# postworthy/ghost

Measured on AMD Instinct MI355X. Metric: swapped frames/sec at 256×256 bf16, 1/2/4/8 MI355X; AAD decoder HBM GB/s, higher is better.
Workload: dtype bf16; 1 GPU; BASELINE config 2: batch=64 synthetic 256x256 aligned faces per GPU, AEI_Net unet num_blocks=2, faceshifter_batch (u8 in -> u8 out, device-resident; D2H in legs.d2h); global_batch=64, per_gpu_batch=64, backbone=unet, num_blocks=2, identities=1, parallelism=dp1, batches_in_flight=2

## Files before the change

ghost_amd/csrc/conv_halo.hip:

```cpp
#include <cstdio>
#include <cstdlib>
#include <type_traits>
#include <utility>

#include "conv_halo.h"
#include "ghost_common.h"
#include "plan_log.h"

namespace ghost {

template <int TH_, int TW_, int WM_, int WN_, int IMG_ = 1>
struct HaloCfg {
  static constexpr int TH = TH_, TW = TW_, WM = WM_, WN = WN_, IMG = IMG_;
  static constexpr int BN = 64 * WN, NW = WM * WN, WPI = WM / IMG;
  static constexpr int HWW = TW + 2, HHH = TH + 2;
  static constexpr int HIMG = HHH * HWW;
  static constexpr int HP = IMG * HIMG;
  static constexpr int HPIECES = (HP + 15) / 16;
  static constexpr int WPIECES = 9 * BN / 16;
  static constexpr int HALO_B = HPIECES * 1024;
  static constexpr int LDS_B = HALO_B + 9 * BN * 64;
  static constexpr int HPW = (HPIECES + NW - 1) / NW;
  static constexpr int WPW = (WPIECES + NW - 1) / NW;
  static_assert(IMG * TH * TW == 64 * WM, "each wave owns 64 output pixels");
// ... 408 lines not shown
    for (int i = 0; i < 4; ++i) acc[j][i] = f32x4{0.f, 0.f, 0.f, 0.f};

  constexpr bool W16 = !EPX && NCB == 2 && IMG == 1 && !(DBG & 16);
  constexpr int LPITCH = 136, LWAVE = 64 * LPITCH;
  constexpr bool LDSW = !EPX && !W16 && IMG == 1 && !RESW && !(DBG & 16) && STAGE_B >= NW * LWAVE;
  const bool plain = !a.scale && !a.shift && a.slope == 1.f && !a.tanh_out;
  constexpr int NST = ((DBG & 48) || EPX) ? 0 : ((W16 || LDSW) ? 8 : 16) + (STATS ? 1 : 0);
  if (nmine == 0) return;
  constexpr bool SPREAD = (DBG & 4096) == 0;
  constexpr int NPIECE = HPW + (RESW ? 0 : WPW);
  static_assert(NPIECE <= 16, "the spread-issue switch below has sixteen cases");
  constexpr int PPT = 2;
  Tile cur = tile_of(0);
  set_dma_tile(cur);
  issue(lds0, 0);
  __builtin_amdgcn_s_waitcnt(0x0F70);
  int k = 0;
  auto step = [&](const unsigned char* buf, unsigned char* nbuf, auto cbt) {
    constexpr int cb = decltype(cbt)::value;
    if constexpr (cb == 0)
      __builtin_amdgcn_s_waitcnt(((NST >> 4) << 14) | 0x0F70 | (NST & 15));
    else
      __builtin_amdgcn_s_waitcnt(0x0F70);
    __builtin_amdgcn_s_waitcnt(0xC07F);
    __builtin_amdgcn_s_barrier();
    const bool more = cb + 1 < NCB || k + 1 < nmine;
    if constexpr (cb + 1 < NCB) {
      if constexpr (!SPREAD) issue(nbuf, cb + 1);
    } else if (k + 1 < nmine) {
      set_dma_tile(tile_of(k + 1));
      if constexpr (!SPREAD) issue(nbuf, 0);
    }
    constexpr int ncb_next = cb + 1 < NCB ? cb + 1 : 0;
    const unsigned char* wb = RESW ? wres + cb * WBLK_B : buf + HALO_B;
    v8_t<T> wf[2][4], pf[2][4];
    auto load_frags = [&](int tap, v8_t<T> (&w)[4], v8_t<T> (&p)[4]) {
      const int dy = tap / 3, dx = tap - dy * 3;
#pragma unroll
      for (int j = 0; j < 4; ++j) {
        const int n = j * 16 + lr;
        w[j] = *reinterpret_cast<const v8_t<T>*>(wb + (tap * 64 + n) * 64 + ((lq ^ hswz(n)) * 16));
      }
#pragma unroll
      for (int i = 0; i < 4; ++i) {
        const int q = i * 16 + lr;
        const int P = G::himg(wid) + (G::hrow0(wid) + q / TW + dy) * HWW + q % TW + dx;
        p[i] = *reinterpret_cast<const v8_t<T>*>(buf + P * 64 + ((lq ^ hswz(P)) * 16));
      }
    };
    if constexpr ((DBG & 8) == 0) {
      load_frags(0, wf[0], pf[0]);
      if constexpr ((DBG & 64) != 0) load_frags(1, wf[1], pf[1]);
      asm volatile("" ::: "memory");
#pragma unroll
      for (int tap = 0; tap < 9; ++tap) {
        if constexpr ((DBG & 128) == 0) __builtin_amdgcn_s_waitcnt(0xC07F);
        if (tap + 1 < 9 && (DBG & 64) == 0) load_frags(tap + 1, wf[(tap + 1) & 1], pf[(tap + 1) & 1]);
#pragma unroll
        for (int j = 0; j < 4; ++j)
#pragma unroll
          for (int i = 0; i < 4; ++i)
            acc[j][i] = mfma16x16x32<T>(wf[tap & 1][j], pf[tap & 1][i], acc[j][i]);
        if constexpr (SPREAD) {
          if (more) {
            pp_unroll(std::make_integer_sequence<int, 16>{}, [&](auto qt) {
              constexpr int q = decltype(qt)::value;
              const int pc = tap * PPT + q;
              if ((q < PPT || (tap == 8 && pc < NPIECE)) && pc < NPIECE) {
                switch (pc) {
#define GHOST_SPREAD_CASE(N) case N: if constexpr (N < NPIECE) issue_piece(nbuf, ncb_next, std::integral_constant<int, N>{}); break;
                  GHOST_SPREAD_CASE(0) GHOST_SPREAD_CASE(1) GHOST_SPREAD_CASE(2) GHOST_SPREAD_CASE(3)
                  GHOST_SPREAD_CASE(4) GHOST_SPREAD_CASE(5) GHOST_SPREAD_CASE(6) GHOST_SPREAD_CASE(7)
                  GHOST_SPREAD_CASE(8) GHOST_SPREAD_CASE(9) GHOST_SPREAD_CASE(10) GHOST_SPREAD_CASE(11)
                  GHOST_SPREAD_CASE(12) GHOST_SPREAD_CASE(13) GHOST_SPREAD_CASE(14) GHOST_SPREAD_CASE(15)
#undef GHOST_SPREAD_CASE
                  default: break;
                }
              }
            });
          }
        }
        if constexpr ((DBG & 128) == 0) {
          if (tap + 1 < 9 && (DBG & 64) == 0) {
            __builtin_amdgcn_sched_group_barrier(0x100, 8, 0);
            __builtin_amdgcn_sched_group_barrier(0x008, 16, 0);
          } else {
            __builtin_amdgcn_sched_group_barrier(0x008, 16, 0);
          }
          __builtin_amdgcn_sched_barrier(0);
        } else {
          asm volatile("" ::: "memory");
        }
      }
    }
    if constexpr (cb + 1 < NCB) return;
    if constexpr ((DBG & 32) != 0) {
      float t = 0.f;
#pragma unroll
      for (int j = 0; j < 4; ++j)
#pragma unroll
        for (int i = 0; i < 4; ++i) {
          t += acc[j][i][0] + acc[j][i][1] + acc[j][i][2] + acc[j][i][3];
          acc[j][i] = f32x4{0.f, 0.f, 0.f, 0.f};
        }
      if (__float_as_uint(t) == 0x7fc00123u) ay_[lane] = (T)t;
      return;
    }
    unsigned char* stg = const_cast<unsigned char*>(buf) + wid * LWAVE;
    if constexpr (LDSW) {
      __builtin_amdgcn_s_waitcnt(0xC07F);
      __builtin_amdgcn_s_barrier();
    }
    auto epi_body = [&](auto mt) {
    constexpr int MODE = decltype(mt)::value;
    const bool has_res = MODE == 1 || (MODE == 0 && ares_ != nullptr);
    uint2 rraw[4][4];
    if (has_res) {
#pragma unroll
      for (int i = 0; i < 4; ++i) {
        const int q = i * 16 + lr;
        const int oy = cur.y0 + G::hrow0(wid) + q / TW, ox = cur.x0 + q % TW;
        const long pix = cur.base + (long)G::img(wid) * a.H * a.W + (long)oy * a.W + ox;
        const bool in = !EPX || (oy < a.H && ox < a.W);
#pragma unroll
        for (int j = 0; j < 4; ++j)
          rraw[i][j] = in ? *reinterpret_cast<const uint2*>(ares_ + pix * a.ldres + cur.n0 + j * 16 + lq * 4)
                          : make_uint2(0u, 0u);
      }
    }
#pragma unroll
    for (int i = 0; i < 4; ++i) {
      const int q = i * 16 + lr;
      const int oy = cur.y0 + G::hrow0(wid) + q / TW, ox = cur.x0 + q % TW;
      const long pix = cur.base + (long)G::img(wid) * a.H * a.W + (long)oy * a.W + ox;
      uint2 ov[4];
      if constexpr (EPX) {
        if (oy >= a.H || ox >= a.W) {
#pragma unroll
          for (int j = 0; j < 4; ++j) acc[j][i] = f32x4{0.f, 0.f, 0.f, 0.f};
          continue;
        }
      }
#pragma unroll
      for (int j = 0; j < 4; ++j) {
        const int n = cur.n0 + j * 16 + lq * 4;
        float rv[4] = {0.f, 0.f, 0.f, 0.f};
        if (has_res) {
          const T* e = reinterpret_cast<const T*>(&rraw[i][j]);
#pragma unroll
          for (int r = 0; r < 4; ++r) rv[r] = (float)e[r];
        }
        uint2 o;
        T* oe = reinterpret_cast<T*>(&o);
        if constexpr (EPX) {
          const f32x4 tsc = *reinterpret_cast<const f32x4*>(s_sc + n);
          const f32x4 tsh = *reinterpret_cast<const f32x4*>(s_sh + n);
          const f32x4 tpr = *reinterpret_cast<const f32x4*>(s_ex + n);
          float v[4];
#pragma unroll
          for (int r = 0; r < 4; ++r) {
            float t = fmaf(acc[j][i][r], tsc[r], tsh[r]);
            if (a.res_first) t += rv[r];
            t = t > 0.f ? t : t * tpr[r];
            if (!a.res_first) t += rv[r];
            if (a.tanh_out) t = tanhf(t);
            v[r] = t;
            oe[r] = (T)t;
            acc[j][i][r] = 0.f;
          }
          *reinterpret_cast<uint2*>(ay_ + pix * a.ldy + n) = o;
          if (ay2_) {
            const f32x4 tsc2 = *reinterpret_cast<const f32x4*>(s_ex + NMAX + n);
            const f32x4 tsh2 = *reinterpret_cast<const f32x4*>(s_ex + 2 * NMAX + n);
#pragma unroll
            for (int r = 0; r < 4; ++r) oe[r] = (T)(v[r] * tsc2[r] + tsh2[r]);
            *reinterpret_cast<uint2*>(ay2_ + pix * a.ldy2 + n) = o;
          }
        } else {
        float v[4];
        if constexpr (MODE != 0) {
#pragma unroll
          for (int r = 0; r < 4; ++r) v[r] = MODE == 1 ? acc[j][i][r] + rv[r] : acc[j][i][r];
        } else {
          const f32x4 tsc = *reinterpret_cast<const f32x4*>(s_sc + n);
          const f32x4 tsh = *reinterpret_cast<const f32x4*>(s_sh + n);
#pragma unroll
          for (int r = 0; r < 4; ++r) {
            float t = fmaf(acc[j][i][r], tsc[r], tsh[r]);
            t = t > 0.f ? t : t * a.slope;
            t += rv[r];
            if (a.tanh_out) t = tanhf(t);
            v[r] = t;
          }
        }
        o.x = pack2<T>(v[0], v[1]);
        o.y = pack2<T>(v[2], v[3]);
        if constexpr (STATS) {
          const f32x2 a01 = unpack2<T>(o.x), a23 = unpack2<T>(o.y);
          acc[j][i] = f32x4{a01.x, a01.y, a23.x, a23.y};
        } else {
          acc[j][i] = f32x4{0.f, 0.f, 0.f, 0.f};
        }
        if constexpr (W16) ov[j] = o;
        else if constexpr (LDSW) {
          *reinterpret_cast<uint2*>(stg + q * LPITCH + 32 * j + 8 * lq) = o;
        }
        else if constexpr (!(DBG & 16)) *reinterpret_cast<uint2*>(ay_ + pix * a.ldy + n) = o;
        else if ((o.x ^ o.y) == 0x7fc00001u) *reinterpret_cast<uint2*>(ay_ + pix * a.ldy + n) = o;
        }
      }
      if constexpr (W16) {
        uint2 a0, a1, b0, b1;
        {
          const auto x0 = __builtin_amdgcn_permlane16_swap(ov[0].x, ov[1].x, false, false);
          const auto y0 = __builtin_amdgcn_permlane16_swap(ov[0].y, ov[1].y, false, false);
          const auto x1 = __builtin_amdgcn_permlane16_swap(ov[2].x, ov[3].x, false, false);
          const auto y1 = __builtin_amdgcn_permlane16_swap(ov[2].y, ov[3].y, false, false);
          a0 = make_uint2(x0[0], y0[0]);
          a1 = make_uint2(x0[1], y0[1]);
          b0 = make_uint2(x1[0], y1[0]);
          b1 = make_uint2(x1[1], y1[1]);
        }
        static_assert(G::TW % 16 == 0, "a pixel fragment lies in one tile row");
        const long p0 = pix - lr + (lr & 7);
        store_rows16<T>(ay_ + cur.n0, p0 * a.ldy, (p0 + 8) * a.ldy, lr, (lq >> 1) + 2 * (lq & 1),
                        u32x4{a0.x, a0.y, a1.x, a1.y}, u32x4{b0.x, b0.y, b1.x, b1.y});
      }
    }
    };
    if constexpr (EPX) {
      epi_body(std::integral_constant<int, 0>{});
    } else {
      if (plain) {
        if (ares_) epi_body(std::integral_constant<int, 1>{});
        else epi_body(std::integral_constant<int, 2>{});
      } else {
        epi_body(std::integral_constant<int, 0>{});
      }
    }
    if constexpr (LDSW) {
      asm volatile("" ::: "memory");
      const int c = lane & 7, q0 = lane >> 3;
      T* __restrict__ yw = ay_ + (cur.base + (long)(cur.y0 + G::hrow0(wid)) * a.W + cur.x0) * a.ldy + cur.n0;
      const int lo = q0 * a.ldy + c * 8;
#pragma unroll
      for (int st = 0; st < 8; ++st) {
        const int q = 8 * st + q0;
        const u32x4 v = *reinterpret_cast<const u32x4*>(stg + q * LPITCH + c * 16);
        *reinterpret_cast<u32x4*>(yw + ((st >> 2) * a.W + 8 * (st & 3)) * a.ldy + lo) = v;
      }
    }
    if constexpr (STATS) {
      float S1, S2;
      tile_stats64_1p(acc, lr, S1, S2);
      const int c = cur.n0 + (lr >> 2) * 16 + lq * 4 + (lr & 3);
      float* dst;
      if constexpr (IMG > 1) {
        const long b = cur.base / ((long)a.H * a.W) + G::img(wid);
        dst = a.in_part + (b * (long)a.N + c) * 2;
      } else {
        const int tile = (cur.y0 / G::TH) * a.tiles_x + cur.x0 / TW;
        const long b = cur.base / ((long)a.H * a.W);
        dst = a.in_part + ((((b * a.tiles_x * a.tiles_y) + tile) * 8 + wid) * (long)a.N + c) * 2;
      }
      *reinterpret_cast<float2*>(dst) = make_float2(S1, S2);
    }
  };
  for (; k < nmine; ++k) {
    pp_unroll(std::make_integer_sequence<int, NCB / 2>{}, [&](auto pt) {
      constexpr int P = decltype(pt)::value;
      step(lds0, lds1, std::integral_constant<int, 2 * P>{});
      step(lds1, lds0, std::integral_constant<int, 2 * P + 1>{});
    });
    if (k + 1 < nmine) cur = tile_of(k + 1);
  }
  asm volatile("s_waitcnt vmcnt(0)" ::: "memory");
}

template <int BN>
struct HaloTCfg {
  static constexpr int TIH = 8, TIW = 16;
  static constexpr int HWW = TIW + 2, HP = (TIH + 2) * HWW;
  static constexpr int HPIECES = (HP + 15) / 16;
  static constexpr int WPIECES = 16 * BN / 16;
  static constexpr int HALO_B = HPIECES * 1024;
  static constexpr int LDS_B = HALO_B + 16 * BN * 64;
  static constexpr int NW = 8;
  static constexpr int HPW = (HPIECES + NW - 1) / NW;
  static constexpr int WPW = (WPIECES + NW - 1) / NW;
  static constexpr int TN = BN / 16;
};

struct HaloTArgs {
  const void* x;
  const void* w;
  void* y;
  const float* scale;
  const float* shift;
  const void* res;
  long wpar;
  int H, W, Cin, ldx, N, Kpad, ldy, ldres;
  float slope;
  int tiles_x, tiles_y, nNt;
};

template <typename T, int BN>
__global__ void __launch_bounds__(512) __attribute__((amdgpu_waves_per_eu(4, 8))) convT_halo_kernel(const HaloTArgs a) {
  const T* __restrict__ ax_ = reinterpret_cast<const T*>(a.x);
  const T* __restrict__ aw_ = reinterpret_cast<const T*>(a.w);
  T* __restrict__ ay_ = reinterpret_cast<T*>(a.y);
  const T* __restrict__ ares_ = reinterpret_cast<const T*>(a.res);
  using G = HaloTCfg<BN>;
  constexpr int HWW = G::HWW, HP = G::HP, HPIECES = G::HPIECES, WPIECES = G::WPIECES, HALO_B = G::HALO_B;
  constexpr int NWAVES = G::NW, HPW = G::HPW, WPW = G::WPW, TN = G::TN;
  __shared__ __attribute__((aligned(1024))) unsigned char lds[G::LDS_B];
  const int tid = threadIdx.x, lane = tid & 63, lr = lane & 15, lq = lane >> 4, wid = tid >> 6;
  const int ph = wid >> 1, py = ph >> 1, px = ph & 1, hf = wid & 1;
  int t = xcd_tile(blockIdx.x, gridDim.x);
  const int nt = t % a.nNt;
  t /= a.nNt;
  const int tx = t % a.tiles_x;
  t /= a.tiles_x;
  const int ty = t % a.tiles_y;
  const int b = t / a.tiles_y;
  const int y0 = ty * G::TIH, x0 = tx * G::TIW, n0 = nt * BN;
  const T* __restrict__ xs = ax_ + (long)b * a.H * a.W * a.ldx;

  const int prow = lane >> 2, slot = lane & 3;
  int h_off[HPW];
  unsigned h_ok = 0u;
#pragma unroll
  for (int j = 0; j < HPW; ++j) {
    const int piece = wid + j * NWAVES;
    const int P = piece * 16 + prow;
    const int hy = P / HWW, hx = P - hy * HWW;
    const int iy = y0 - 1 + hy, ix = x0 - 1 + hx;
    const bool ok = piece < HPIECES && P < HP && iy >= 0 && iy < a.H && ix >= 0 && ix < a.W;
    h_off[j] = ok ? (iy * a.W + ix) * a.ldx + ((slot ^ hswz(P)) * 8) : 0;
    h_ok |= (ok ? 1u : 0u) << j;
  }
  const T* wsrc[WPW];
#pragma unroll
  for (int j = 0; j < WPW; ++j) {
    const int piece = wid + j * NWAVES;
    const int pt = piece / (BN / 16), n = (piece % (BN / 16)) * 16 + prow;
    wsrc[j] = aw_ + (pt >> 2) * a.wpar + (long)(n0 + n) * a.Kpad + (pt & 3) * 32 + ((slot ^ hswz(n)) * 8);
  }

  f32x4 acc[TN][4];
#pragma unroll
  for (int j = 0; j < TN; ++j)
#pragma unroll
    for (int i = 0; i < 4; ++i) acc[j][i] = f32x4{0.f, 0.f, 0.f, 0.f};

  const int ncb = a.Cin / 32;
  for (int cb = 0; cb < ncb; ++cb) {
#if defined(__HIP_DEVICE_COMPILE__)
#pragma unroll
    for (int j = 0; j < HPW; ++j) {
      const int piece = wid + j * NWAVES;
      if (piece < HPIECES) {
        const void* src = ((h_ok >> j) & 1u) ? (const void*)(xs + h_off[j] + cb * 32) : (const void*)g_halo_zero;
        __builtin_amdgcn_global_load_lds(src, lds + piece * 1024, 16, 0, 0);
      }
    }
#pragma unroll
    for (int j = 0; j < WPW; ++j) {
      const int piece = wid + j * NWAVES;
      if (piece < WPIECES) __builtin_amdgcn_global_load_lds(wsrc[j] + cb * 128, lds + HALO_B + piece * 1024, 16, 0, 0);
    }
#endif
    asm volatile("s_waitcnt vmcnt(0)" ::: "memory");
    __syncthreads();
#pragma unroll
    for (int tp = 0; tp < 4; ++tp) {
      asm volatile("" ::: "memory");
      const int dy = py - (tp >> 1), dx = px - (tp & 1);
      v8_t<T> wf[TN], pf[4];
#pragma unroll
      for (int j = 0; j < TN; ++j) {
        const int n = j * 16 + lr;
        wf[j] = *reinterpret_cast<const v8_t<T>*>(lds + HALO_B + ((ph * 4 + tp) * BN + n) * 64 + ((lq ^ hswz(n)) * 16));
      }
#pragma unroll
      for (int i = 0; i < 4; ++i) {
        const int P = (hf * 4 + i + 1 + dy) * HWW + lr + 1 + dx;
        pf[i] = *reinterpret_cast<const v8_t<T>*>(lds + P * 64 + ((lq ^ hswz(P)) * 16));
      }
#pragma unroll
      for (int j = 0; j < TN; ++j)
#pragma unroll
        for (int i = 0; i < 4; ++i) acc[j][i] = mfma16x16x32<T>(wf[j], pf[i], acc[j][i]);
    }
    __syncthreads();
  }

  const int Wo = 2 * a.W, Ho = 2 * a.H;
#pragma unroll
  for (int i = 0; i < 4; ++i) {
    const int oy = 2 * (y0 + hf * 4 + i) + py, ox = 2 * (x0 + lr) + px;
    const long pix = ((long)b * Ho + oy) * Wo + ox;
#pragma unroll
    for (int j = 0; j < TN; ++j) {
      const int n = n0 + j * 16 + lq * 4;
      if (n >= a.N) continue;
      float rv[4] = {0.f, 0.f, 0.f, 0.f};
      if (ares_) {
        const uint2 raw = *reinterpret_cast<const uint2*>(ares_ + pix * a.ldres + n);
        const T* e = reinterpret_cast<const T*>(&raw);
#pragma unroll
        for (int r = 0; r < 4; ++r) rv[r] = (float)e[r];
      }
      uint2 o;
      T* oe = reinterpret_cast<T*>(&o);
#pragma unroll
      for (int r = 0; r < 4; ++r) {
        float v = acc[j][i][r];
        if (a.scale) v *= a.scale[n + r];
        if (a.shift) v += a.shift[n + r];
        v = v > 0.f ? v : v * a.slope;
        oe[r] = (T)(v + rv[r]);
      }
      *reinterpret_cast<uint2*>(ay_ + pix * a.ldy + n) = o;
    }
  }
}

bool convT_halo_supported(const ConvDesc& d) {
  static const int enabled = GHOST_KNOB("GHOST_CONVT_HALO", 1);
  if (!enabled || d.kind != CONV_T4S2 || !is16(d.ti) || d.to != d.ti || d.epi != EPI_STD) return false;
  if (d.u8 || d.tanh_out || d.force_split || d.Cin % 32 || d.ldx % 8 || d.ldy % 4 || (d.res && d.ldres % 4)) return false;
  if (d.res_first || d.prelu || d.y2) return false;
  if (d.Hi % HaloTCfg<64>::TIH || d.Wi % HaloTCfg<64>::TIW || d.Kpad < 4 * d.Cin) return false;
  if (!(d.N % 64 == 0 || d.N == 32) || d.Npad < d.N) return false;
  if ((uintptr_t)d.x % 16 || (uintptr_t)d.w % 16 || (uintptr_t)d.y % 8 || (d.res && (uintptr_t)d.res % 8)) return false;
  {
    const int bn = d.N == 32 ? 32 : 64;
    const long nt = (long)d.B * (d.Hi / HaloTCfg<64>::TIH) * (d.Wi / HaloTCfg<64>::TIW) * ((d.N + bn - 1) / bn);
    if (nt < 128) return false;
  }
  return (long)d.Hi * d.Wi * d.ldx < (1L << 31);
}

PlanSig convT_halo_signature(const ConvDesc& d) {
  PlanSig g;
  snprintf(g.s, sizeof(g.s), "convT_halo t=%s BN=%d Cin=%d N=%d res=%d", plan_dt(d.ti), d.N == 32 ? 32 : 64, d.Cin, d.N,
           d.res != nullptr);
  return g;
}

template <typename T, int BN>
static int haloT_launch(const ConvDesc& d, hipStream_t s) {
  HaloTArgs a{};
  a.x = d.x; a.w = d.w; a.y = d.y;
  a.scale = d.scale; a.shift = d.shift; a.res = d.res;
  a.wpar = (long)d.Npad * d.Kpad;
  a.H = d.Hi; a.W = d.Wi; a.Cin = d.Cin; a.ldx = d.ldx; a.N = d.N; a.Kpad = d.Kpad;
  a.ldy = d.ldy; a.ldres = d.ldres; a.slope = d.slope;
  a.tiles_x = d.Wi / HaloTCfg<BN>::TIW; a.tiles_y = d.Hi / HaloTCfg<BN>::TIH; a.nNt = (d.N + BN - 1) / BN;
  const long ntiles = (long)d.B * a.tiles_x * a.tiles_y * a.nNt;
  GHOST_PLAN_LOG("%s", convT_halo_signature(d).s);
  hipLaunchKernelGGL((convT_halo_kernel<T, BN>), dim3((unsigned)ntiles), dim3(512), 0, s, a);
  return (int)hipGetLastError();
}

int convT_halo(const ConvDesc& d, hipStream_t s) {
  if (!convT_halo_supported(d)) return -1;
  if (d.ti == GHOST_F16) return d.N == 32 ? haloT_launch<_Float16, 32>(d, s) : haloT_launch<_Float16, 64>(d, s);
  return d.N == 32 ? haloT_launch<bf16, 32>(d, s) : haloT_launch<bf16, 64>(d, s);
}

struct HaloGeom { int TH, TW, IMG, NW; const char* name; };
template <class G> static constexpr HaloGeom halo_geom(const char* name) { return {G::TH, G::TW, G::IMG, G::NW, name}; }
static constexpr HaloGeom kHaloGeom[] = {halo_geom<HaloWide>("Wide"), halo_geom<HaloSmall>("Small"),
                                         halo_geom<HaloImg8>("Img8"), halo_geom<HaloPair>("Pair")};

HaloPlan halo_plan(const ConvDesc& d, int ncu) {
  HaloPlan p;
  static const int enabled = GHOST_KNOB("GHOST_CONV_HALO", 1);
  if (!enabled || d.kind != CONV_FWD || d.kh != 3 || d.kw != 3 || d.stride != 1 || d.pad != 1) return p;
  if (!is16(d.ti) || d.to != d.ti || d.epi != EPI_STD || d.u8 || d.force_split) return p;
  if (d.Cin % 32 || d.ldx % 8 || d.N % 64 || d.ldy % 4 || (d.res && d.ldres % 4)) return p;
  if (d.y2 && (d.ldy2 % 4 || (uintptr_t)d.y2 % 8 || !d.scale2 || !d.shift2)) return p;
  const bool wide = d.Wi % HaloWide::TW == 0 && d.Hi % HaloWide::TH == 0;
  const long stx = (d.Wi + HaloSmall::TW - 1) / HaloSmall::TW, sty = (d.Hi + HaloSmall::TH - 1) / HaloSmall::TH;
  const bool small_ok = 4L * d.Hi * d.Wi >= 3L * stx * sty * HaloSmall::TW * HaloSmall::TH;
  const int ncb = d.Cin / 32;
  const bool ncb_pow2 = ncb == 2 || ncb == 4 || ncb == 8 || ncb == 16 || ncb == 32;
  const bool plain = !d.prelu && !d.y2 && !d.res_first;
  const bool w16 = d.ldy % 8 == 0 && (uintptr_t)d.y % 16 == 0;
  static const int img8_on = GHOST_KNOB("GHOST_HALO_IMG8", 1);
  const bool img8 = img8_on && d.Hi == HaloImg8::TH && d.Wi == HaloImg8::TW && d.B % HaloImg8::IMG == 0 && d.N <= 1024 &&
                    plain && !d.tanh_out && d.Cin % 64 == 0 && d.Cin <= 1024 && ncb_pow2 && w16;
  if ((!wide && !small_ok && !img8) || d.Kpad < 9 * d.Cin || d.Npad < d.N) return p;
  if ((uintptr_t)d.x % 16 || (uintptr_t)d.w % 16 || (uintptr_t)d.y % 8 || (d.res && (uintptr_t)d.res % 8)) return p;
  if ((long)d.Hi * d.Wi * d.ldx >= (1L << 31) || (long)d.Npad * d.Kpad >= (1L << 31)) return p;
  if (!img8) {
    const int th = wide ? HaloWide::TH : HaloSmall::TH, tw = wide ? HaloWide::TW : HaloSmall::TW;
    const long items = (long)d.B * ((d.Hi + th - 1) / th) * ((d.Wi + tw - 1) / tw) * (d.N / 64);
    static const int min_items = GHOST_KNOB("GHOST_HALO_MIN_ITEMS", 64);
    if (items < min_items) return p;
  }
  static const int max_n = GHOST_KNOB("GHOST_CONV_HALO_MAXN", 1 << 30);
  if (d.N > max_n) return p;

  static const int pp = GHOST_KNOB("GHOST_HALO_PP", 1);
  static const int max_cin = GHOST_KNOB("GHOST_HALO_PP_MAXCIN", 1024);
  static const int force_small = GHOST_KNOB("GHOST_HALO_PP_SMALL", 0);
  const bool cin_ok = d.Cin == 64 || d.Cin == 128 || d.Cin == 192 || d.Cin == 256 || d.Cin == 512 || d.Cin == 1024;
  if (img8) {
    p.kernel = HaloKernel::HaloPP; p.tile = HaloTile::Img8;
    p.nrec = 1;
  } else if (wide && pp && plain && w16 && d.N <= 512 && cin_ok && d.Cin <= max_cin && !d.tanh_out) {
    p.kernel = HaloKernel::HaloPP; p.tile = HaloTile::Wide;
    p.nrec = (d.Hi / HaloWide::TH) * (d.Wi / HaloWide::TW) * 8;
  } else if (pp && !wide && small_ok && (force_small || d.Wi % HaloSmall::TW || d.Hi % HaloSmall::TH || !plain) &&
             d.N <= 512 && d.Cin % 64 == 0 && (ncb_pow2 || ncb == 6)) {
    static const int pair = GHOST_KNOB("GHOST_HALO_PAIR", 1);
    const long pair_items = (long)(d.B / 2) * stx * sty * (d.N / 64);
    p.kernel = HaloKernel::HaloPP;
    p.tile = pair && d.B % 2 == 0 && d.N <= 256 && pair_items >= ncu ? HaloTile::Pair : HaloTile::Small;
  } else {
    p.kernel = HaloKernel::Halo;
    p.tile = wide ? HaloTile::Wide : HaloTile::Small;
  }
  const HaloGeom& g = kHaloGeom[(int)p.tile];
  p.tiles_x = (d.Wi + g.TW - 1) / g.TW; p.tiles_y = (d.Hi + g.TH - 1) / g.TH;
  p.ntiles = d.B / g.IMG * p.tiles_x * p.tiles_y * (d.N / 64);
  p.block = (unsigned)g.NW * 64;
  if (p.kernel == HaloKernel::HaloPP) {
    p.resw = d.Cin <= 64 && d.N == 64;
    p.ncb = ncb;
    p.stats = d.in_part && p.nrec > 0;
    static const int pct = GHOST_KNOB("GHOST_PP_GRID_PCT", 100);
    const int gcu = pct >= 100 ? ncu : (ncu * pct / 100 + 7) / 8 * 8;
    p.grid = (unsigned)(p.ntiles < gcu ? p.ntiles : gcu);
  } else {
    p.grid = (unsigned)p.ntiles;
  }
  return p;
}

bool conv3x3_halo_supported(const ConvDesc& d) { return halo_plan(d, 256).kernel != HaloKernel::None; }

bool conv3x3_pp_takes(const ConvDesc& d, int* nrec) {
  const HaloPlan p = halo_plan(d, 256);
  if (p.nrec > 0 && nrec) *nrec = p.nrec;
  return p.nrec > 0;
}

PlanSig halo_signature(const HaloPlan& p, const ConvDesc& d) {
  const HaloGeom& g = kHaloGeom[(int)p.tile];
  const int overhang = d.Hi % g.TH != 0 || d.Wi % g.TW != 0;
  PlanSig sig;
  if (p.kernel == HaloKernel::HaloPP)
    snprintf(sig.s, sizeof(sig.s), "halo_pp t=%s tile=%s RESW=%d STATS=%d NCB=%d N=%d overhang=%d uneven=%d", plan_dt(d.ti),
             g.name, (int)p.resw, (int)p.stats, p.ncb, d.N, overhang, p.ntiles % (int)p.grid != 0);
  else
    snprintf(sig.s, sizeof(sig.s), "halo t=%s tile=%s Cin=%d N=%d overhang=%d", plan_dt(d.ti), g.name, d.Cin, d.N, overhang);
  return sig;
}

typedef void (*HaloFn)(const HaloArgs);
struct HaloRow {
  HaloKernel kernel;
  HaloTile tile;
  bool resw, stats;
  int ncb;
  HaloFn fn;
};

template <typename T>
static HaloFn halo_fn(const HaloPlan& p) {
#define GHOST_ROW(G, r, st, nb) {HaloKernel::HaloPP, HaloTile::G, r, st, nb, conv3x3_halo_pp_kernel<T, Halo##G, r, st, nb>},
#define GHOST_PP(G, st)                                                                             \
  GHOST_ROW(G, true, st, 2) GHOST_ROW(G, false, st, 2) GHOST_ROW(G, false, st, 4) GHOST_ROW(G, false, st, 6) \
  GHOST_ROW(G, false, st, 8) GHOST_ROW(G, false, st, 16) GHOST_ROW(G, false, st, 32)
  static const HaloRow rows[] = {
      {HaloKernel::Halo, HaloTile::Wide, false, false, 0, conv3x3_halo_kernel<T, HaloWide>},
      {HaloKernel::Halo, HaloTile::Small, false, false, 0, conv3x3_halo_kernel<T, HaloSmall>},
      GHOST_PP(Wide, false) GHOST_PP(Wide, true) GHOST_PP(Img8, false) GHOST_PP(Img8, true)
      GHOST_PP(Small, false) GHOST_PP(Pair, false)};
#undef GHOST_PP
#undef GHOST_ROW
  for (const HaloRow& r : rows)
    if (r.kernel == p.kernel && r.tile == p.tile && r.resw == p.resw && r.stats == p.stats && r.ncb == p.ncb) return r.fn;
  return nullptr;
}

static int num_cus() {
  static const int n = [] {
    int dev = 0, v = 0;
    if (hipGetDevice(&dev) != hipSuccess || hipDeviceGetAttribute(&v, hipDeviceAttributeMultiprocessorCount, dev) !=
                                                 hipSuccess || v <= 0)
      v = 256;
    return v;
  }();
  return n;
}

template <typename T>
static int halo_launch(const ConvDesc& d, const HaloPlan& p, hipStream_t s) {
  const HaloFn fn = halo_fn<T>(p);
  if (!fn) return -1;
  HaloArgs a{};
  a.x = d.x; a.w = d.w; a.y = d.y;
  a.scale = d.scale; a.shift = d.shift; a.res = d.res;
  a.H = d.Hi; a.W = d.Wi; a.Cin = d.Cin; a.ldx = d.ldx; a.N = d.N; a.Kpad = d.Kpad;
  a.ldy = d.ldy; a.ldres = d.ldres; a.tanh_out = d.tanh_out; a.slope = d.slope;
  a.prelu = d.prelu; a.y2 = d.y2; a.scale2 = d.scale2; a.shift2 = d.shift2; a.ldy2 = d.ldy2;
  a.res_first = d.res_first;
  a.tiles_x = p.tiles_x; a.tiles_y = p.tiles_y; a.nNt = d.N / 64; a.ntiles = p.ntiles;
  if (p.kernel == HaloKernel::HaloPP) {
    static const int dbg = GHOST_KNOB("GHOST_HALO_DBG", 0);
    a.dbg = dbg;
    a.in_part = d.in_part;
#ifdef GHOST_TUNING
    if (p.tile == HaloTile::Wide && dbg) {
      using G = HaloWide;
      constexpr int NT = G::NW * 64;
      const unsigned g = p.grid;
#define GHOST_PP_DBX(R, NB, V)                                                                                    \
  if (p.resw == R && p.ncb == NB && dbg == V) {                                                                  \
    if (a.in_part)                                                                                               \
      hipLaunchKernelGGL((conv3x3_halo_pp_kernel<T, G, R, true, NB, V>), dim3((unsigned)g), dim3(NT), 0, s, a);  \
    else                                                                                                         \
      hipLaunchKernelGGL((conv3x3_halo_pp_kernel<T, G, R, false, NB, V>), dim3((unsigned)g), dim3(NT), 0, s, a); \
    return (int)hipGetLastError();                                                                               \
  }
      GHOST_PP_DBX(true, 2, 4096) GHOST_PP_DBX(false, 4, 4096) GHOST_PP_DBX(false, 8, 4096)
      GHOST_PP_DBX(true, 2, 2) GHOST_PP_DBX(true, 2, 16) GHOST_PP_DBX(true, 2, 32) GHOST_PP_DBX(true, 2, 34)
      GHOST_PP_DBX(true, 2, 8)
      GHOST_PP_DBX(false, 16, 4096) GHOST_PP_DBX(false, 32, 4096)
#undef GHOST_PP_DBX
    }
#endif
  }
  GHOST_PLAN_LOG("%s", halo_signature(p, d).s);
  hipLaunchKernelGGL(fn, dim3(p.grid), dim3(p.block), 0, s, a);
  return (int)hipGetLastError();
}

int conv3x3_halo(const ConvDesc& d, hipStream_t s) {
  const HaloPlan p = halo_plan(d, num_cus());
  if (p.kernel == HaloKernel::None || (d.in_part && !p.stats)) return -1;
  return d.ti == GHOST_F16 ? halo_launch<_Float16>(d, p, s) : halo_launch<bf16>(d, p, s);
}

}
```

Measured before the change: 11990 frames/s.

## Add persistent double-buffered transposed-conv halo kernel with async LDS prefetch

Adds a persistent variant of the stride-2 transposed-conv halo kernel. It launches at most one block per CU, and each block loops over its share of tiles. Halo and weight pieces for the next channel block or the next tile go through global_load_lds into a second LDS buffer while MFMAs run on the current one. Scale and shift are cached in LDS. This targets load latency and per-tile launch and prologue overhead, at the cost of doubled LDS use, which lowers occupancy, and a more fragile hand-scheduled pipeline.

```diff
diff --git a/ghost_amd/csrc/conv_halo.hip b/ghost_amd/csrc/conv_halo.hip
--- a/ghost_amd/csrc/conv_halo.hip
+++ b/ghost_amd/csrc/conv_halo.hip
@@ -734,6 +734,7 @@
   int H, W, Cin, ldx, N, Kpad, ldy, ldres;
   float slope;
   int tiles_x, tiles_y, nNt;
+  int ntiles;
 };
 
 template <typename T, int BN>
@@ -858,21 +859,257 @@
   }
 }
 
-bool convT_halo_supported(const ConvDesc& d) {
+constexpr int kConvTPPMaxN = 128;
+
+GHOST_DEV float convT_epi(float v, float sc, float sh, float slope) {
+#pragma clang fp contract(off)
+  v = v * sc;
+  v = v + sh;
+  return v > 0.f ? v : v * slope;
+}
+
+template <typename T, int BN, int DBG = 0>
+__global__ void __launch_bounds__(512) convT_halo_pp_kernel(const HaloTArgs a) {
+  const T* __restrict__ ax_ = reinterpret_cast<const T*>(a.x);
+  const T* __restrict__ aw_ = reinterpret_cast<const T*>(a.w);
+  T* __restrict__ ay_ = reinterpret_cast<T*>(a.y);
+  const T* __restrict__ ares_ = reinterpret_cast<const T*>(a.res);
+  using G = HaloTCfg<BN>;
+  constexpr int HWW = G::HWW, HP = G::HP, HPIECES = G::HPIECES, WPIECES = G::WPIECES, HALO_B = G::HALO_B;
+  constexpr int NW = G::NW, HPW = G::HPW, WPW = G::WPW, TN = G::TN, STAGE_B = G::LDS_B, NMAX = kConvTPPMaxN;
+  static_assert(WPIECES == WPW * NW, "every wave stages WPW weight pieces");
+  static_assert(2 * STAGE_B + 2 * NMAX * (int)sizeof(float) < 160 * 1024, "two stages and the channel tables in 160 KB of LDS");
+  __shared__ __attribute__((aligned(1024))) unsigned char lds0[STAGE_B];
+  __shared__ __attribute__((aligned(1024))) unsigned char lds1[STAGE_B];
+  __shared__ __attribute__((aligned(16))) float s_sc[NMAX], s_sh[NMAX];
+  const int tid = threadIdx.x, lane = tid & 63, lr = lane & 15, lq = lane >> 4,
+            wid = __builtin_amdgcn_readfirstlane(tid >> 6);
+  const int ph = wid >> 1, py = ph >> 1, px = ph & 1, hf = wid & 1;
+  const int prow = lane >> 2, slot = lane & 3;
+
+  const int G_ = gridDim.x;
+  const int xt = xcd_tile(blockIdx.x, G_);
+  const int nmine = a.ntiles > xt ? (a.ntiles - xt + G_ - 1) / G_ : 0;
+  if (nmine == 0) return;
+  const int ncb = a.Cin / 32;
+  for (int n = tid; n < a.N && n < NMAX; n += NW * 64) {
+    s_sc[n] = a.scale ? a.scale[n] : 1.f;
+    s_sh[n] = a.shift ? a.shift[n] : -0.f;
+  }
+
+  struct Tile { int b, y0, x0, n0; };
+  auto tile_of = [&](int k) {
+    int t = k * G_ + xt;
+    Tile r;
+    const int nt = t % a.nNt;
+    t /= a.nNt;
+    const int tx = t % a.tiles_x;
+    t /= a.tiles_x;
+    const int ty = t % a.tiles_y;
+    r.b = t / a.tiles_y;
+    r.y0 = ty * G::TIH;
+    r.x0 = tx * G::TIW;
+    r.n0 = nt * BN;
+    return r;
+  };
+  int h_off[HPW];
+  unsigned h_ok = 0u;
+  long dma_x = 0, dma_w = 0;
+  auto set_dma_tile = [&](const Tile& t) {
+    dma_x = (long)t.b * a.H * a.W * a.ldx;
+    dma_w = (long)t.n0 * a.Kpad;
+    h_ok = 0u;
+#pragma unroll
+    for (int j = 0; j < HPW; ++j) {
+      const int piece = wid + j * NW;
+      const int P = piece * 16 + prow;
+      const int hy = P / HWW, hx = P - hy * HWW;
+      const int iy = t.y0 - 1 + hy, ix = t.x0 - 1 + hx;
+      const bool ok = piece < HPIECES && P < HP && iy >= 0 && iy < a.H && ix >= 0 && ix < a.W;
+      h_off[j] = ok ? (iy * a.W + ix) * a.ldx + ((slot ^ hswz(P)) * 8) : 0;
+      h_ok |= (ok ? 1u : 0u) << j;
+    }
+  };
+  int w_off[WPW];
+#pragma unroll
+  for (int j = 0; j < WPW; ++j) {
+    const int piece = wid + j * NW;
+    const int pt = piece / (BN / 16), n = (piece % (BN / 16)) * 16 + prow;
+    w_off[j] = (pt >> 2) * (int)a.wpar + n * a.Kpad + (pt & 3) * 32 + ((slot ^ hswz(n)) * 8);
+  }
+  constexpr int NPIECE = HPW + WPW;
+  auto issue_piece = [&](unsigned char* buf, int cb, auto jt) {
+    constexpr int jj = decltype(jt)::value;
+#if defined(__HIP_DEVICE_COMPILE__)
+    if constexpr (jj < HPW) {
+      const int piece = wid + jj * NW;
+      if (piece < HPIECES && !(DBG & 2)) {
+        const T* __restrict__ xs = ax_ + dma_x + cb * 32;
+        const void* src = ((h_ok >> jj) & 1u) ? (const void*)(xs + h_off[jj]) : (const void*)g_halo_zero;
+        __builtin_amdgcn_global_load_lds(src, buf + piece * 1024, 16, 0, 0);
+      }
+    } else if constexpr (!(DBG & 4)) {
+      constexpr int j = jj - HPW;
+      const T* __restrict__ ws = aw_ + dma_w + cb * 128;
+      __builtin_amdgcn_global_load_lds(ws + w_off[j], buf + HALO_B + (wid + j * NW) * 1024, 16, 0, 0);
+    }
+#endif
+  };
+
+  f32x4 acc[TN][4];
+#pragma unroll
+  for (int j = 0; j < TN; ++j)
+#pragma unroll
+    for (int i = 0; i < 4; ++i) acc[j][i] = f32x4{0.f, 0.f, 0.f, 0.f};
+
+  set_dma_tile(tile_of(0));
+  pp_unroll(std::make_integer_sequence<int, NPIECE>{}, [&](auto jt) { issue_piece(lds0, 0, jt); });
+  int k = 0, cb = 0;
+  constexpr int PPT = (NPIECE + 3) / 4;
+  const int Wo = 2 * a.W, Ho = 2 * a.H;
+
+  auto step = [&](const unsigned char* buf, unsigned char* nbuf) {
+    __builtin_amdgcn_s_waitcnt(0x0F70);
+    __builtin_amdgcn_s_waitcnt(0xC07F);
+    __builtin_amdgcn_s_barrier();
+    const bool last_cb = cb + 1 == ncb;
+    const bool more = !last_cb || k + 1 < nmine;
+    const int cb_next = last_cb ? 0 : cb + 1;
+    if (last_cb && k + 1 < nmine) set_dma_tile(tile_of(k + 1));
+    f32x4 tsc[TN], tsh[TN];
+    Tile cur{};
+    if (last_cb) {
+      cur = tile_of(k);
+#pragma unroll
+      for (int j = 0; j < TN; ++j) {
+        tsc[j] = *reinterpret_cast<const f32x4*>(s_sc + cur.n0 + j * 16 + lq * 4);
+        tsh[j] = *reinterpret_cast<const f32x4*>(s_sh + cur.n0 + j * 16 + lq * 4);
+      }
+    }
+    asm volatile("" ::: "memory");
+    if constexpr ((DBG & 8) == 0) {
+      v8_t<T> wf[2][TN], pf[2][4];
+      auto load_frags = [&](int tp, v8_t<T> (&w)[TN], v8_t<T> (&p)[4]) {
+        const int dy = py - (tp >> 1), dx = px - (tp & 1);
+#pragma unroll
+        for (int j = 0; j < TN; ++j) {
+          const int n = j * 16 + lr;
+          w[j] = *reinterpret_cast<const v8_t<T>*>(buf + HALO_B + ((ph * 4 + tp) * BN + n) * 64 + ((lq ^ hswz(n)) * 16));
+        }
+#pragma unroll
+        for (int i = 0; i < 4; ++i) {
+          const int P = (hf * 4 + i + 1 + dy) * HWW + lr + 1 + dx;
+          p[i] = *reinterpret_cast<const v8_t<T>*>(buf + P * 64 + ((lq ^ hswz(P)) * 16));
+        }
+      };
+      load_frags(0, wf[0], pf[0]);
+      asm volatile("" ::: "memory");
+      pp_unroll(std::make_integer_sequence<int, 4>{}, [&](auto tpt) {
+        constexpr int tp = decltype(tpt)::value;
+        __builtin_amdgcn_s_waitcnt(0xC07F);
+        if constexpr (tp + 1 < 4) load_frags(tp + 1, wf[(tp + 1) & 1], pf[(tp + 1) & 1]);
+#pragma unroll
+        for (int j = 0; j < TN; ++j)
+#pragma unroll
+          for (int i = 0; i < 4; ++i) acc[j][i] = mfma16x16x32<T>(wf[tp & 1][j], pf[tp & 1][i], acc[j][i]);
+        if (more) {
+          pp_unroll(std::make_integer_sequence<int, PPT>{}, [&](auto qt) {
+            constexpr int pc = tp * PPT + decltype(qt)::value;
+            if constexpr (pc < NPIECE) issue_piece(nbuf, cb_next, std::integral_constant<int, pc>{});
+          });
+        }
+        if constexpr (tp + 1 < 4) {
+          __builtin_amdgcn_sched_group_barrier(0x100, TN + 4, 0);
+          __builtin_amdgcn_sched_group_barrier(0x008, 4 * TN, 0);
+        } else {
+          __builtin_amdgcn_sched_group_barrier(0x008, 4 * TN, 0);
+        }
+        __builtin_amdgcn_sched_barrier(0);
+      });
+    } else {
+      if (more) pp_unroll(std::make_integer_sequence<int, NPIECE>{}, [&](auto jt) { issue_piece(nbuf, cb_next, jt); });
+    }
+    if (!last_cb) {
+      ++cb;
+      return;
+    }
+    auto epi = [&](auto rest) {
+      constexpr bool RES = decltype(rest)::value;
+      uint2 rraw[4][TN];
+      if constexpr (RES) {
+#pragma unroll
+        for (int i = 0; i < 4; ++i) {
+          const int oy = 2 * (cur.y0 + hf * 4 + i) + py, ox = 2 * (cur.x0 + lr) + px;
+          const long pix = ((long)cur.b * Ho + oy) * Wo + ox;
+#pragma unroll
+          for (int j = 0; j < TN; ++j)
+            rraw[i][j] = *reinterpret_cast<const uint2*>(ares_ + pix * a.ldres + cur.n0 + j * 16 + lq * 4);
+        }
+      }
+#pragma unroll
+      for (int i = 0; i < 4; ++i) {
+        const int oy = 2 * (cur.y0 + hf * 4 + i) + py, ox = 2 * (cur.x0 + lr) + px;
+        const long pix = ((long)cur.b * Ho + oy) * Wo + ox;
+#pragma unroll
+        for (int j = 0; j < TN; ++j) {
+          const int n = cur.n0 + j * 16 + lq * 4;
+          float rv[4] = {0.f, 0.f, 0.f, 0.f};
+          if constexpr (RES) {
+            const T* e = reinterpret_cast<const T*>(&rraw[i][j]);
+#pragma unroll
+            for (int r = 0; r < 4; ++r) rv[r] = (float)e[r];
+          }
+          uint2 o;
+          T* oe = reinterpret_cast<T*>(&o);
+#pragma unroll
+          for (int r = 0; r < 4; ++r) oe[r] = (T)(convT_epi(acc[j][i][r], tsc[j][r], tsh[j][r], a.slope) + rv[r]);
+          *reinterpret_cast<uint2*>(ay_ + pix * a.ldy + n) = o;
+          acc[j][i] = f32x4{0.f, 0.f, 0.f, 0.f};
+        }
+      }
+    };
+    if (ares_) epi(std::true_type{});
+    else epi(std::false_type{});
+    ++k;
+    cb = 0;
+  };
+
+  while (k < nmine) {
+    step(lds0, lds1);
+    if (k < nmine) step(lds1, lds0);
+  }
+  asm volatile("s_waitcnt vmcnt(0)" ::: "memory");
+}
+
+struct ConvTPlan {
+  bool ok = false, pp = false;
+  int bn = 64, tiles_x = 0, tiles_y = 0, nNt = 0, ntiles = 0;
+  unsigned grid = 0;
+};
+
+static ConvTPlan convT_plan(const ConvDesc& d, int ncu) {
+  ConvTPlan p;
   static const int enabled = GHOST_KNOB("GHOST_CONVT_HALO", 1);
-  if (!enabled || d.kind != CONV_T4S2 || !is16(d.ti) || d.to != d.ti || d.epi != EPI_STD) return false;
-  if (d.u8 || d.tanh_out || d.force_split || d.Cin % 32 || d.ldx % 8 || d.ldy % 4 || (d.res && d.ldres % 4)) return false;
-  if (d.res_first || d.prelu || d.y2) return false;
-  if (d.Hi % HaloTCfg<64>::TIH || d.Wi % HaloTCfg<64>::TIW || d.Kpad < 4 * d.Cin) return false;
-  if (!(d.N % 64 == 0 || d.N == 32) || d.Npad < d.N) return false;
-  if ((uintptr_t)d.x % 16 || (uintptr_t)d.w % 16 || (uintptr_t)d.y % 8 || (d.res && (uintptr_t)d.res % 8)) return false;
-  {
-    const int bn = d.N == 32 ? 32 : 64;
-    const long nt = (long)d.B * (d.Hi / HaloTCfg<64>::TIH) * (d.Wi / HaloTCfg<64>::TIW) * ((d.N + bn - 1) / bn);
-    if (nt < 128) return false;
-  }
-  return (long)d.Hi * d.Wi * d.ldx < (1L << 31);
-}
+  if (!enabled || d.kind != CONV_T4S2 || !is16(d.ti) || d.to != d.ti || d.epi != EPI_STD) return p;
+  if (d.u8 || d.tanh_out || d.force_split || d.Cin % 32 || d.ldx % 8 || d.ldy % 4 || (d.res && d.ldres % 4)) return p;
+  if (d.res_first || d.prelu || d.y2) return p;
+  if (d.Hi % HaloTCfg<64>::TIH || d.Wi % HaloTCfg<64>::TIW || d.Kpad < 4 * d.Cin) return p;
+  if (!(d.N % 64 == 0 || d.N == 32) || d.Npad < d.N) return p;
+  if ((uintptr_t)d.x % 16 || (uintptr_t)d.w % 16 || (uintptr_t)d.y % 8 || (d.res && (uintptr_t)d.res % 8)) return p;
+  p.bn = d.N == 32 ? 32 : 64;
+  p.tiles_x = d.Wi / HaloTCfg<64>::TIW; p.tiles_y = d.Hi / HaloTCfg<64>::TIH; p.nNt = (d.N + p.bn - 1) / p.bn;
+  const long nt = (long)d.B * p.tiles_y * p.tiles_x * p.nNt;
+  if (nt < 128 || nt >= (1L << 31)) return p;
+  if ((long)d.Hi * d.Wi * d.ldx >= (1L << 31)) return p;
+  p.ok = true;
+  p.ntiles = (int)nt;
+  static const int pp = GHOST_KNOB("GHOST_CONVT_PP", 1);
+  p.pp = pp && d.N <= kConvTPPMaxN && d.Cin >= 32 && 4L * d.Npad * d.Kpad < (1L << 31);
+  p.grid = (unsigned)(p.pp && p.ntiles > ncu ? ncu : p.ntiles);
+  return p;
+}
+
+bool convT_halo_supported(const ConvDesc& d) { return convT_plan(d, 256).ok; }
 
 PlanSig convT_halo_signature(const ConvDesc& d) {
   PlanSig g;
@@ -881,25 +1118,37 @@
   return g;
 }
 
+static int num_cus();
+
 template <typename T, int BN>
-static int haloT_launch(const ConvDesc& d, hipStream_t s) {
+static int haloT_launch(const ConvDesc& d, const ConvTPlan& p, hipStream_t s) {
   HaloTArgs a{};
   a.x = d.x; a.w = d.w; a.y = d.y;
   a.scale = d.scale; a.shift = d.shift; a.res = d.res;
   a.wpar = (long)d.Npad * d.Kpad;
   a.H = d.Hi; a.W = d.Wi; a.Cin = d.Cin; a.ldx = d.ldx; a.N = d.N; a.Kpad = d.Kpad;
   a.ldy = d.ldy; a.ldres = d.ldres; a.slope = d.slope;
-  a.tiles_x = d.Wi / HaloTCfg<BN>::TIW; a.tiles_y = d.Hi / HaloTCfg<BN>::TIH; a.nNt = (d.N + BN - 1) / BN;
-  const long ntiles = (long)d.B * a.tiles_x * a.tiles_y * a.nNt;
+  a.tiles_x = p.tiles_x; a.tiles_y = p.tiles_y; a.nNt = p.nNt; a.ntiles = p.ntiles;
   GHOST_PLAN_LOG("%s", convT_halo_signature(d).s);
-  hipLaunchKernelGGL((convT_halo_kernel<T, BN>), dim3((unsigned)ntiles), dim3(512), 0, s, a);
+  if (p.pp) {
+#ifdef GHOST_TUNING
+    static const int dbg = GHOST_KNOB("GHOST_CONVT_DBG", 0);
+    if (dbg == 6) hipLaunchKernelGGL((convT_halo_pp_kernel<T, BN, 6>), dim3(p.grid), dim3(512), 0, s, a);
+    else if (dbg == 8) hipLaunchKernelGGL((convT_halo_pp_kernel<T, BN, 8>), dim3(p.grid), dim3(512), 0, s, a);
+    else
+#endif
+    hipLaunchKernelGGL((convT_halo_pp_kernel<T, BN>), dim3(p.grid), dim3(512), 0, s, a);
+  } else {
+    hipLaunchKernelGGL((convT_halo_kernel<T, BN>), dim3(p.grid), dim3(512), 0, s, a);
+  }
   return (int)hipGetLastError();
 }
 
 int convT_halo(const ConvDesc& d, hipStream_t s) {
-  if (!convT_halo_supported(d)) return -1;
-  if (d.ti == GHOST_F16) return d.N == 32 ? haloT_launch<_Float16, 32>(d, s) : haloT_launch<_Float16, 64>(d, s);
-  return d.N == 32 ? haloT_launch<bf16, 32>(d, s) : haloT_launch<bf16, 64>(d, s);
+  const ConvTPlan p = convT_plan(d, num_cus());
+  if (!p.ok) return -1;
+  if (d.ti == GHOST_F16) return p.bn == 32 ? haloT_launch<_Float16, 32>(d, p, s) : haloT_launch<_Float16, 64>(d, p, s);
+  return p.bn == 32 ? haloT_launch<bf16, 32>(d, p, s) : haloT_launch<bf16, 64>(d, p, s);
 }
 
 struct HaloGeom { int TH, TW, IMG, NW; const char* name; };
```

New measurement: 11980 frames/s, median of 2. No clear change (-0.0%).
